# dfm/emcee

Measured on AMD Instinct MI355X. Metric: walker-updates/sec (whole node), 64-dim correlated Gaussian, StretchMove a=2, higher is better.
Workload: dtype f64

## Files before the change

### emcee_amd/csrc/emx.hip

```cpp
#include <hip/hip_runtime.h>

#include <dlfcn.h>

#include <algorithm>
#include <chrono>
#include <cmath>
#include <cstdint>
#include <cstdio>
#include <cstring>
#include <deque>
#include <mutex>
#include <string>
#include <type_traits>
#include <vector>

#include "../../include/emx.h"
#include "emx_internal.hpp"
#include "emx_kernels.hpp"
#include "emx_launch.hpp"
#include "emx_mtdev.hpp"
#include "emx_mtjump.hpp"
#include "emx_mtpipe.hpp"
#include "emx_walkkde.hpp"
#include "emx_rng.hpp"
// ... 287 lines not shown
    } ring[PLAN_RING + MTDEV_SLOTS];
    MtPlanPipeline* pipe = nullptr;
    int64_t pipe_taken = 0;
    int pipe_ring0 = 0;
    int pipe_nsinks = PIPE_SINKS;
    std::deque<int64_t> pipe_uploads;
    bool pipe_defer = false;
    std::vector<std::pair<int64_t, int>> pipe_deferred;
    hipEvent_t pipe_batch_ev[8] = {};
    int pipe_batch_n = 0, pipe_cons_n = 0;
    unsigned long long* pipe_done = nullptr;
    unsigned* pipe_arrived = nullptr;
    hipStream_t up_stream = nullptr;
    int64_t tune_mt_device_finish = 1;
    int64_t tune_persist_exact_mix = 1;
    int64_t pipe_raw_steps = 0;
    int64_t tune_mt_pipeline = -1;
    MtDevProducer* mtdev = nullptr;
    int64_t mtdev_taken = 0;
    int64_t tune_persist_local = 1;
    int64_t tune_persist_exact_max = 32768;
    int64_t tune_persist_exact_regen_max = 131072;
    int64_t tune_persist_exact_steps = 16;
    int64_t tune_fetch_avoid = 1;
    int64_t tune_fetch_blocks = 64;
    bool pipe_fetch_local = false;
    int64_t tune_fetch_delay_us = 0;
    int64_t tune_persist_span = 1;
    int64_t tune_persist_mix = 1;
    int persist_mix_fits = -1;
    int64_t tune_persist_slab = 1;
    int64_t persist_slab_launches = 0;
    int64_t tune_persist_rows_late = 1;
    int64_t tune_persist_stagger = -1;
    int64_t tune_persist_max_halfsteps = PERSIST_MAX_ITERS;
    int64_t tune_mt_device_min_regen = 786432;
    int64_t tune_mt_regen_min = 16384;
    int64_t pipe_regen_steps = 0;
    int64_t tune_persist_odd = 1;
    int64_t tune_persist_slab_skew = 1;
    int64_t tune_persist_slab_local_max = 4096;
    int64_t call_steps = 1;
    int64_t tune_persist_exact = 1;
    int64_t tune_persist_valu = 1;
    int64_t tune_persist_local_max = 8192;
    int64_t tune_slab = 1;
    int64_t tune_slab_skew = 1;
    int64_t tune_mt_device = 1;
    int64_t tune_mt_device_min = 147456;
    int64_t tune_mt_lookahead = 2;
    int64_t tune_mt_tok_wshift = 11, tune_mt_tok_tail = 2048;
    int64_t mtdev_steps_total = 0, mtdev_starts = 0;
    bool mtdev_defer_release = false;
    int64_t mtdev_release_pending = -1;
    MtDevStats mtdev_stats_last;
    int ring_pos = 0;
    struct Prepared {
        int move, S, slot;
        bool lean;
        int gcol;
        uint64_t step;
        NativeArgs nat;
        double cursor_before;
    };
    std::deque<Prepared> prepared;
    int64_t prep_hint = 1;
// ... 1037 lines not shown
        return 0;
    }
    if (!strcmp(key, "persist_slab_skew")) {
        c->tune_persist_slab_skew = v < 0 ? 0 : (v > 4 ? 4 : v);
        return 0;
    }
    if (!strcmp(key, "persist_slab_local_max_walkers")) {
        c->tune_persist_slab_local_max = v;
        return 0;
    }
    if (!strcmp(key, "persist_odd")) {
        c->tune_persist_odd = v ? 1 : 0;
        return 0;
    }
    if (!strcmp(key, "persist_exact_regen_max_walkers")) {
        PIPE_STOP(c);
        c->tune_persist_exact_regen_max = v;
        return 0;
    }
    if (!strcmp(key, "mt_device_min_walkers_regen")) {
        PIPE_STOP(c);
        c->tune_mt_device_min_regen = v;
        return 0;
    }
    if (!strcmp(key, "mt_regen_min_walkers")) {
        PIPE_STOP(c);
        c->tune_mt_regen_min = v < 0 ? 0 : v;
        return 0;
    }
    if (!strcmp(key, "persist_rows_late")) {
        c->tune_persist_rows_late = v < 0 ? 0 : v > 2 ? 2 : v;
        return 0;
    }
    if (!strcmp(key, "persist_stagger")) {
        c->tune_persist_stagger = v < 0 ? -1 : v > 1279 ? 1279 : v;
        return 0;
    }
    if (!strcmp(key, "persist_max_halfsteps")) {
        c->tune_persist_max_halfsteps = v;
        return 0;
    }
    if (!strcmp(key, "persist_slab")) {
        c->tune_persist_slab = (v == 1 || v == 2) ? v : 0;
        return 0;
    }
    if (!strcmp(key, "persist_local")) {
        c->tune_persist_local = v ? 1 : 0;
        return 0;
    }
    if (!strcmp(key, "persist_exact")) {
        PIPE_STOP(c);
        c->tune_persist_exact = v ? 1 : 0;
        return 0;
    }
    if (!strcmp(key, "persist_exact_max_walkers")) {
        PIPE_STOP(c);
        c->tune_persist_exact_max = v;
        return 0;
    }
    if (!strcmp(key, "persist_exact_steps")) {
        c->tune_persist_exact_steps = std::max<int64_t>(1, std::min<int64_t>(v, 16));
        return 0;
    }
    if (!strcmp(key, "fetch_blocks")) {
        c->tune_fetch_blocks = std::max<int64_t>(0, std::min<int64_t>(v, 65536));
        return 0;
// ... 1628 lines not shown
    const int64_t own = N / nsplits;
    if ((own % 16) != 0) return 0;
    const int64_t tiles = own / 16, per_xcd = std::min<int64_t>(32, std::max<int64_t>(1, cu / 8));
    for (int wpb = 1; wpb <= 8; wpb <<= 1)
        if ((tiles % wpb) == 0 && tiles / wpb <= per_xcd) return tiles / wpb >= 2 ? wpb : 0;
    return 0;
}
static bool persist_local_ok(const emx_ctx* c, const emx_move_desc& m) {
    const bool known = ((m.kind == EMX_MOVE_STRETCH || m.kind == EMX_MOVE_DE) && m.nsplits == 2) || (m.kind == EMX_MOVE_SNOOKER && m.nsplits == 4);
    const int64_t lmax = (c->target == EMX_TARGET_DENSE_GAUSS && c->Dp > 64) ? std::min(c->tune_persist_local_max, c->tune_persist_slab_local_max)
                                                                               : c->tune_persist_local_max;
    return c->tune_persist_local != 0 && known && c->N <= lmax &&
           persist_shape_local_of(c->N, m.nsplits, c->num_cu) != 0;
}
static int persist_shape(const emx_ctx* c, int nsplits) { return persist_shape_of(c->N, nsplits, c->num_cu); }
static bool persist_valu_shape(const Shape& sh) {
    return (sh.G == 8 && (sh.CH == 1 || sh.CH == 2 || sh.CH == 4)) || (sh.G == 4 && sh.CH == 1) || (sh.G == 16 && sh.V == 1 && sh.CH == 4);
}
static bool persist_slab_ok(const emx_ctx* c) {
    if (!c->tune_persist_slab || c->target != EMX_TARGET_DENSE_GAUSS || dense_is_wide(c) || c->Dp < 80 || c->Dp > 128) return false;
    if (c->tune_persist_slab != 2 && c->Dp >= 112 && c->N / 2 / 16 >= 8 * (int64_t)c->num_cu && !(c->D & 1)) return false;
    const Shape sh = pick_shape(c->D, c->Dp);
    return (sh.G == 16 && sh.V == 2 && sh.CH == 4) || (c->tune_persist_odd != 0 && sh.G == 32 && sh.V == 1 && sh.CH == 4);
}

static bool persist_grid_fits(const emx_ctx* cc, const emx_move_desc& m, int wpb) {
    emx_ctx* c = const_cast<emx_ctx*>(cc);
    if (m.kind < 0 || m.kind > 3) return false;
    if (c->persist_fits[m.kind] < 0) {
        const int64_t groups = c->N / m.nsplits / 16 / wpb;
        int per_cu = 0;
        const hipError_t e = c->Dp > 64 ? persist_slab_occupancy(c->Dp / 16, m.kind, c->D & 1, 64 * wpb, slab_lds_bytes(c->Dp, wpb), &per_cu)
                             : (c->D & 1) ? persist_dense_odd_occupancy(c->Dp / 16, m.kind, 64 * wpb, dense_lds_bytes(c->Dp, wpb), &per_cu)
                                        : hot_persist_occupancy(c->Dp / 16, m.kind, 64 * wpb, dense_lds_bytes(c->Dp, wpb), &per_cu);
        c->persist_fits[m.kind] = (e != hipSuccess || (int64_t)per_cu * c->num_cu >= groups) ? 1 : 0;
    }
    return c->persist_fits[m.kind] != 0;
}

static bool persist_valu_wide_ok(const emx_ctx* c, const emx_move_desc& m) {
    const bool known = ((m.kind == EMX_MOVE_STRETCH || m.kind == EMX_MOVE_DE) && m.nsplits == 2) || (m.kind == EMX_MOVE_SNOOKER && m.nsplits == 4);
    const bool valu = c->target == EMX_TARGET_ISO_GAUSS || c->target == EMX_TARGET_DIAG_GAUSS || c->target == EMX_TARGET_ROSENBROCK || c->target == EMX_TARGET_BOX;
    const int64_t nmax = (regen_ctx_ok(c) && m.kind == EMX_MOVE_STRETCH) ? std::max(c->tune_persist_exact_max, c->tune_persist_exact_regen_max) : c->tune_persist_exact_max;
    return known && valu && c->rng_mode == EMX_RNG_MT19937 && c->tune_persist_valu != 0 && c->N <= nmax && persist_shape(c, m.nsplits) != 0;
}

static bool persist_move_ok(const emx_ctx* c, const emx_move_desc& m) {
    const bool known = ((m.kind == EMX_MOVE_STRETCH || m.kind == EMX_MOVE_DE) && m.nsplits == 2) || (m.kind == EMX_MOVE_SNOOKER && m.nsplits == 4);
    if (!known) return false;
    if (c->target == EMX_TARGET_DENSE_GAUSS && c->Dp > 64 && (m.kind == EMX_MOVE_SNOOKER || !persist_slab_ok(c))) return false;
    if (c->target == EMX_TARGET_DENSE_GAUSS && c->Dp > 64 && (c->D & 1) && m.kind != EMX_MOVE_STRETCH) return false;
    if (persist_local_ok(c, m)) return true;
    if (c->target != EMX_TARGET_DENSE_GAUSS) return persist_valu_wide_ok(c, m);
    const int wpb = persist_shape(c, m.nsplits);
    return wpb != 0 && persist_grid_fits(c, m, wpb);
}

static bool persist_mix_member(const emx_move_desc& m) {
    return (m.kind == EMX_MOVE_DE && m.nsplits == 2) || (m.kind == EMX_MOVE_SNOOKER && m.nsplits == 4);
}
static bool persist_mix_local(const emx_ctx* c) {
    for (const auto& m : c->moves)
        if (persist_mix_member(m) && !persist_local_ok(c, m)) return false;
    return persist_shape_local_of(c->N, 2, c->num_cu) != 0;
}
static bool persist_mix_ok(const emx_ctx* cc) {
    emx_ctx* c = const_cast<emx_ctx*>(cc);
// ... 321 lines not shown
        if (mtmode && !devp && c->cur.slot >= 0) used_slots.push_back(c->cur.slot);
        rc = emx_step_end(c);
        if (rc) return rc;
        ++steps;
    }
    if (mtmode && !devp) {
        c->pipe_fetch_local = launch_local;
        const int rcf = pipe_fetch_deferred(c);
        if (rcf) return rcf;
    }
    c->pipe_defer = false;
    if (launch_mix) grid = dim3((unsigned)(c->N / 2 / 16 / c->persist_wpb));
    if (launch_local) grid.x *= 8;
    if (grid.x != c->persist_grid) {
        HIPOK(c, hipMemsetAsync(c->persist_bar, 0, PERSIST_BAR_WORDS * sizeof(unsigned), c->stream));
        c->persist_epoch = 0;
        c->persist_lepoch = 0;
        c->persist_hepoch = 0;
        c->persist_grid = grid.x;
    }
    P.niter = n;
    P.bar = c->persist_bar;
    P.started_host = c->persist_started;
    P.ver = c->persist_ver;
    P.epoch0 = c->persist_epoch + (unsigned)c->tune_persist_test_skew;
    P.lepoch0 = c->persist_lepoch;
    P.hepoch0 = c->persist_hepoch + (unsigned)c->tune_persist_test_skew;
    if (launch_local) {
        c->persist_lepoch += (unsigned)(n - 1);
        c->persist_hepoch += 1u;
    }
    P.timeout_ticks = 100000000ull * (unsigned long long)std::max<int64_t>(1, c->tune_persist_timeout_ms) / 1000ull;
    const bool fam_dense64 = c->target == EMX_TARGET_DENSE_GAUSS && c->Dp <= 64;
    P.stagger = c->tune_persist_stagger >= 0 ? (int32_t)c->tune_persist_stagger
                : (launch_local || store || !fam_dense64) ? 0
                : (launch_mix || launch_move == EMX_MOVE_DE) ? 528
                : launch_move == EMX_MOVE_STRETCH ? 516 : 0;
    c->persist_epoch += (unsigned)n;
    P.seq = ++c->persist_seq;
    lg.seq = P.seq;
    lg.steps = steps;
    if (!mtmode || (!devp && lg.pipe_id != nullptr)) c->plog.push_back(lg);
    hipEvent_t e0 = nullptr, e1 = nullptr;
    const bool prof = c->prof_max > 0 && c->prof_n < c->prof_max;
    if (prof) {
        e0 = c->prof[2 * c->prof_n];
        e1 = c->prof[2 * c->prof_n + 1];
    }
    {
        std::lock_guard<std::mutex> lk(g_persist_mu);
        const int dev = c->device;
        if (dev >= 0 && dev < MAX_DEVICES) {
            if (!g_persist_ev[dev]) HIPOK(c, hipEventCreateWithFlags(&g_persist_ev[dev], hipEventDisableTiming));
            if (g_persist_last[dev] && g_persist_last[dev] != c) HIPOK(c, hipStreamWaitEvent(c->stream, g_persist_ev[dev], 0));
        }
        if (prof) HIPOK(c, hipEventRecord(e0, c->stream));
        hipError_t e;
        const bool rows_late = store && (c->tune_persist_rows_late == 2 ||
                                         (c->tune_persist_rows_late == 1 && (launch_local || c->N / 2 / 16 >= 8 * (int64_t)c->num_cu)));
        if (c->target != EMX_TARGET_DENSE_GAUSS) {
            const Shape shv = pick_shape(c->D, c->D);
            e = launch_persist_valu(shv.G, shv.V, shv.CH, launch_move, launch_local ? 1 : 0, grid, block, c->stream, P);
        } else if (launch_mix) {
            e = launch_persist_mix(c->Dp / 16, launch_local ? 1 : 0, grid, block, lds, c->stream, P);
        } else if (c->Dp > 64) {
            P.base.ablate = c->tune_persist_slab_skew ? 256 | (int32_t)((c->tune_persist_slab_skew - 1) << 9) : 0;
            e = launch_persist_slab(c->Dp / 16, launch_move, launch_local ? 1 : 0, c->D & 1, grid, block, lds, c->stream, P);
            c->persist_slab_launches++;
        } else if (c->D & 1) {
            e = launch_persist_dense_odd(c->Dp / 16, launch_move, launch_local ? 1 : 0, grid, block, lds, c->stream, P);
        } else {
            e = launch_hot_persist_dense(c->Dp / 16, launch_move, launch_local ? 1 : 0, rows_late ? 1 : 0, grid, block, lds, c->stream, P);
        }
        if (launch_local) c->persist_local_launches++;
        if (e != hipSuccess) FAIL(c, -2, "persistent half-step launch failed: %s", hipGetErrorString(e));
        if (prof) {
            HIPOK(c, hipEventRecord(e1, c->stream));
            c->prof_n++;
        }
        if (dev >= 0 && dev < MAX_DEVICES) {
            HIPOK(c, hipEventRecord(g_persist_ev[dev], c->stream));
            g_persist_last[dev] = c;
        }
    }
    if (!used_slots.empty()) {
        hipEvent_t& ev = c->pipe_batch_ev[4 + (c->pipe_cons_n & 3)];
        if (!ev) HIPOK(c, hipEventCreateWithFlags(&ev, hipEventDisableTiming));
        c->pipe_cons_n++;
        HIPOK(c, hipEventRecord(ev, c->stream));
        for (int sl : used_slots) {
            c->ring[sl].consumed_ref = ev;
            c->ring[sl].busy = true;
            c->ring[sl].last_seq = P.seq;
        }
    }
    if (mtmode && !devp) pipe_poll(c);
    c->mtdev_defer_release = false;
    if (c->mtdev_release_pending >= 0 && c->mtdev) {
        const int rcr = c->mtdev->release_batch(c->mtdev_release_pending, c->stream);
        c->mtdev_release_pending = -1;
        if (rcr) FAIL(c, rcr, "%s", c->mtdev->error().c_str());
    }
    c->persist_launches++;
    c->persist_halfsteps += n;
    *done = steps;
// ... 1597 lines not shown
```

### emcee_amd/csrc/emx_hot.hip

```cpp
#include "emx_launch.hpp"

namespace emx {

hipError_t launch_hot_stretch_dense64(int lean, dim3 grid, dim3 block, size_t lds, hipStream_t st, const HalfStepArgs& a) {
    if (lean == 2) return launch_one<8, 2, 4, MOVE_STRETCH, 4, 2>(grid, block, lds, st, a);
    if (lean == 3) return launch_one<8, 2, 4, MOVE_STRETCH, 4, 3>(grid, block, lds, st, a);
    if (lean == 4) return launch_one<8, 2, 4, MOVE_STRETCH, 4, 4>(grid, block, lds, st, a);
    return launch_one<8, 2, 4, MOVE_STRETCH, 4, 1>(grid, block, lds, st, a);
}

template <int G, int V, int CH, int DPB, int MOVE, bool LOCAL = false, bool ROWS_LATE = false>
static hipError_t launch_persist(dim3 grid, dim3 block, size_t lds, hipStream_t st, const PersistArgs& P) {
    auto kern = k_persist<G, V, CH, DPB, MOVE, LOCAL, ROWS_LATE>;
    static size_t lds_granted[MAX_DEVICES] = {};
    int dev = 0;
    if (lds > 48 * 1024 && hipGetDevice(&dev) == hipSuccess && dev >= 0 && dev < MAX_DEVICES && lds > lds_granted[dev]) {
        hipError_t e = hipFuncSetAttribute((const void*)kern, hipFuncAttributeMaxDynamicSharedMemorySize, (int)lds);
        if (e != hipSuccess) return e;
        lds_granted[dev] = lds;
    }
    hipLaunchKernelGGL(kern, grid, block, lds, st, P);
    return hipGetLastError();
}

hipError_t launch_hot_persist_dense(int dpb, int move, int local, int rows_late, dim3 grid, dim3 block, size_t lds, hipStream_t st, const PersistArgs& P) {
    if (rows_late && move == MOVE_STRETCH) {
#define EMX_SCASE(b, ch)                                                                                       \
    if (dpb == b)                                                                                              \
        return local ? launch_persist<8, 2, ch, b, MOVE_STRETCH, true, true>(grid, block, lds, st, P)          \
                     : launch_persist<8, 2, ch, b, MOVE_STRETCH, false, true>(grid, block, lds, st, P);
        EMX_SCASE(1, 1) EMX_SCASE(2, 2) EMX_SCASE(3, 4) EMX_SCASE(4, 4)
#undef EMX_SCASE
        return hipErrorInvalidValue;
    }
    if (local) {
#define EMX_LCASE(b, ch)                                                                                           \
    if (dpb == b)                                                                                                  \
        return move == MOVE_DE        ? launch_persist<8, 2, ch, b, MOVE_DE, true>(grid, block, lds, st, P)        \
               : move == MOVE_SNOOKER ? launch_persist<8, 2, ch, b, MOVE_SNOOKER, true>(grid, block, lds, st, P)   \
                                      : launch_persist<8, 2, ch, b, MOVE_STRETCH, true>(grid, block, lds, st, P);
        EMX_LCASE(1, 1) EMX_LCASE(2, 2) EMX_LCASE(3, 4) EMX_LCASE(4, 4)
#undef EMX_LCASE
        return hipErrorInvalidValue;
    }
#define EMX_CASE(b, ch)                                                                                            \
    if (dpb == b)                                                                                                  \
        return move == MOVE_DE        ? launch_persist<8, 2, ch, b, MOVE_DE>(grid, block, lds, st, P)              \
               : move == MOVE_SNOOKER ? launch_persist<8, 2, ch, b, MOVE_SNOOKER>(grid, block, lds, st, P)         \
                                      : launch_persist<8, 2, ch, b, MOVE_STRETCH>(grid, block, lds, st, P);
    EMX_CASE(1, 1) EMX_CASE(2, 2) EMX_CASE(3, 4) EMX_CASE(4, 4)
#undef EMX_CASE
    return hipErrorInvalidValue;
}

template <int G, int V, int CH, int DPB, int MOVE>
static hipError_t persist_occupancy(int threads, size_t lds, int* per_cu) {
    auto kern = k_persist<G, V, CH, DPB, MOVE>;
    if (lds > 48 * 1024) {
        const hipError_t e = hipFuncSetAttribute((const void*)kern, hipFuncAttributeMaxDynamicSharedMemorySize, (int)lds);
        if (e != hipSuccess) return e;
    }
    return hipOccupancyMaxActiveBlocksPerMultiprocessor(per_cu, kern, threads, lds);
}

hipError_t hot_persist_occupancy(int dpb, int move, int threads, size_t lds, int* per_cu) {
#define EMX_CASE(b, ch)                                                                                     \
    if (dpb == b)                                                                                           \
        return move == MOVE_DE        ? persist_occupancy<8, 2, ch, b, MOVE_DE>(threads, lds, per_cu)       \
               : move == MOVE_SNOOKER ? persist_occupancy<8, 2, ch, b, MOVE_SNOOKER>(threads, lds, per_cu)  \
                                      : persist_occupancy<8, 2, ch, b, MOVE_STRETCH>(threads, lds, per_cu);
    EMX_CASE(1, 1) EMX_CASE(2, 2) EMX_CASE(3, 4) EMX_CASE(4, 4)
#undef EMX_CASE
    return hipErrorInvalidValue;
}

hipError_t launch_hot_persist_gauss(int dpb, dim3 grid, dim3 block, size_t lds, hipStream_t st, const PersistGaussArgs& P) {
#define EMX_CASE(b, ch)                                                                                              \
    if (dpb == b) {                                                                                                  \
        auto kern = k_persist_gauss<8, 2, ch, b>;                                                                    \
        static size_t lds_granted[MAX_DEVICES] = {};                                                                 \
        int dev = 0;                                                                                                 \
        if (lds > 48 * 1024 && hipGetDevice(&dev) == hipSuccess && dev >= 0 && dev < MAX_DEVICES && lds > lds_granted[dev]) { \
            hipError_t e = hipFuncSetAttribute((const void*)kern, hipFuncAttributeMaxDynamicSharedMemorySize, (int)lds); \
            if (e != hipSuccess) return e;                                                                           \
            lds_granted[dev] = lds;                                                                                  \
        }                                                                                                            \
        hipLaunchKernelGGL(kern, grid, block, lds, st, P);                                                           \
        return hipGetLastError();                                                                                    \
    }
    EMX_CASE(1, 1) EMX_CASE(2, 2) EMX_CASE(3, 4) EMX_CASE(4, 4)
#undef EMX_CASE
    return hipErrorInvalidValue;
}

}
```

### emcee_amd/csrc/emx_kernels.hpp

```cpp
#pragma once
#include <hip/hip_runtime.h>

#include <cstdint>

#include "emx_planlog.hpp"
#include "emx_rng.hpp"

#ifndef EMX_OPT_RED4
#define EMX_OPT_RED4 1
#endif
#ifndef EMX_OPT_RTILE
#define EMX_OPT_RTILE 1
#endif
#ifndef EMX_LEAN_FOLD_D
#define EMX_LEAN_FOLD_D 0
#endif
#ifndef EMX_LEAN_FOLD_SPW
#define EMX_LEAN_FOLD_SPW 1
#endif
#ifndef EMX_OPT_SKEW
#define EMX_OPT_SKEW 1
#endif
#ifndef EMX_SNOOKER_BUDGET
#define EMX_SNOOKER_BUDGET 48
// ... 989 lines not shown
    const int base = row * D;
    if constexpr (V == 1) {
        typedef unsigned int emx_u2 __attribute__((ext_vector_type(2)));
#pragma unroll
        for (int c = 0; c < CH; ++c) {
            const int d = c * G + gl;
            if (d < D) {
                const emx_u2 w = __builtin_amdgcn_raw_buffer_load_b64(rsrc, (base + d) * 8, 0, CPOL);
                double t;
                __builtin_memcpy(&t, &w, 8);
                r.x[c][0] = t;
            } else {
                r.x[c][0] = 0.0;
            }
        }
        return;
    }
#pragma unroll
    for (int c = 0; c < CH; ++c) {
        const int d = (c * G + gl) * V;
        if (d + 1 < D) {
            const emx_u4 w = __builtin_amdgcn_raw_buffer_load_b128(rsrc, (base + d) * 8, 0, CPOL);
            double2 t;
            __builtin_memcpy(&t, &w, 16);
            r.x[c][0] = t.x;
            r.x[c][1] = t.y;
        } else {
            r.x[c][0] = 0.0;
            r.x[c][1] = 0.0;
        }
    }
}
template <int G, int V, int CH, int CPOL = EMX_CPOL_SC1>
__device__ __forceinline__ void store_row_agent(const Row<G, V, CH>& r, __amdgpu_buffer_rsrc_t rsrc, int row, int D, int gl) {
    static_assert(V == 2 || V == 1, "two coordinates per lane and chunk (even ndim), or one (odd ndim)");
    const int base = row * D;
    if constexpr (V == 1) {
        typedef unsigned int emx_u2 __attribute__((ext_vector_type(2)));
#pragma unroll
        for (int c = 0; c < CH; ++c) {
            const int d = c * G + gl;
            if (d < D) {
                emx_u2 w;
                const double t = r.x[c][0];
                __builtin_memcpy(&w, &t, 8);
                __builtin_amdgcn_raw_buffer_store_b64(w, rsrc, (base + d) * 8, 0, CPOL);
            }
        }
        return;
    }
#pragma unroll
    for (int c = 0; c < CH; ++c) {
        const int d = (c * G + gl) * V;
        if (d + 1 < D) {
            const double2 t = {r.x[c][0], r.x[c][1]};
            emx_u4 w;
            __builtin_memcpy(&w, &t, 16);
            __builtin_amdgcn_raw_buffer_store_b128(w, rsrc, (base + d) * 8, 0, CPOL);
        }
    }
}
template <typename T>
__device__ __forceinline__ void store_agent(T* p, T v) { __hip_atomic_store(p, v, __ATOMIC_RELAXED, __HIP_MEMORY_SCOPE_AGENT); }
__device__ __forceinline__ double load_agent(const double* p) { return __hip_atomic_load(p, __ATOMIC_RELAXED, __HIP_MEMORY_SCOPE_AGENT); }
__device__ __forceinline__ unsigned load_agent(const unsigned* p) { return __hip_atomic_load(p, __ATOMIC_RELAXED, __HIP_MEMORY_SCOPE_AGENT); }
template <bool LOCAL, typename T>
// ... 142 lines not shown
                    }
                } else {
                    o2 = __hip_atomic_fetch_add(gctr, 1u, __ATOMIC_RELAXED, __HIP_MEMORY_SCOPE_AGENT);
                }
                if (open && o2 == k * 8 - 1) {
                    __hip_atomic_store(go + 4, LOCAL ? (xcc & 15u) + 1u : 0u, __ATOMIC_RELAXED, __HIP_MEMORY_SCOPE_AGENT);
                    __hip_atomic_store(go + 3, P.seq, __ATOMIC_RELAXED, __HIP_MEMORY_SCOPE_AGENT);
                    if (P.started_host) __hip_atomic_store(P.started_host, P.seq, __ATOMIC_RELAXED, __HIP_MEMORY_SCOPE_SYSTEM);
                    __hip_atomic_store(go, k, __ATOMIC_RELAXED, __HIP_MEMORY_SCOPE_AGENT);
                }
            }
            const unsigned long long t0 = wall_clock64();
            for (;;) {
                const unsigned long long v = __hip_atomic_load(reinterpret_cast<unsigned long long*>(go), __ATOMIC_RELAXED, __HIP_MEMORY_SCOPE_AGENT);
                if ((v >> 32) != 0ull) {
                    ok = 0;
                    break;
                }
                if ((int)((unsigned)v - k) >= 0) break;
                if (wall_clock64() - t0 > P.timeout_ticks) {
                    raise_status(P.base.status, ST_EXCHANGE_TIMEOUT);
                    __hip_atomic_store(go + 1, 1u, __ATOMIC_RELAXED, __HIP_MEMORY_SCOPE_AGENT);
                    ok = 0;
                    break;
                }
            }
        }
        ok_s = ok;
    }
    __syncthreads();
    return ok_s != 0;
}

template <int G, int V, int CH, int DPB, int MOVE = MOVE_STRETCH, bool LOCAL = false, bool ROWS_LATE = false>
static __global__ __launch_bounds__(512) void k_persist(const PersistArgs P) {
    static_assert(MOVE == MOVE_STRETCH || MOVE == MOVE_DE || MOVE == MOVE_SNOOKER, "the red / blue moves");
    if (LOCAL && (blockIdx.x & 7u) != 0u) return;
    const unsigned bid = LOCAL ? blockIdx.x >> 3 : blockIdx.x, ngroups = LOCAL ? gridDim.x >> 3 : gridDim.x;
    constexpr int CPOL = EMX_CPOL_SC1;
    constexpr int CPOL_ST = LOCAL ? 0 : EMX_CPOL_SC1;
    constexpr bool DE = MOVE == MOVE_DE || MOVE == MOVE_SNOOKER;
    constexpr bool SN = MOVE == MOVE_SNOOKER;
    constexpr bool DEFER = !DE;
    constexpr int WPW = 64 / G;
    constexpr int PPT = 16 / WPW;
    constexpr int PF = PPT;
    static_assert(EMX_OPT_RTILE && EMX_OPT_RED4, "the persistent kernel is the one-tile-per-batch form");
    constexpr int Dp = DPB * 16, KK = Dp / 4, RT = Dp + 2;
    static_assert(G * V * CH >= Dp, "row layout must cover the padded dimension");
    extern __shared__ __attribute__((aligned(16))) double smem[];
    const HalfStepArgs& A = P.base;
    const int lane = threadIdx.x & 63;
    const int wib = threadIdx.x >> 6;
    const int sub = lane / G;
    const int gl = lane % G;
    const int D = A.D;
    double* Sfrag = smem;
    double* muS = smem + dense_img_doubles(Dp);
    double* tile = muS + Dp + (size_t)wib * (16 * RT + 32);
    double* qfS = tile + 16 * RT;
    double* facS = qfS + 16;
    {
        constexpr int IMG2 = (dense_img_doubles(Dp) + Dp) / 2;
        const double2* img = reinterpret_cast<const double2*>(A.tp1);
        double2* dst = reinterpret_cast<double2*>(smem);
        for (int e = threadIdx.x; e < IMG2; e += blockDim.x) dst[e] = img[e];
    }
    Row<G, V, CH> mu;
    load_row<G, V, CH>(mu, A.tp0, D, gl);
// ... 23 lines not shown
    Row<G, V, CH> xi[PF];
    {
        const PersistCols I(P.it[0], (size_t)P.base.N);
        const int pbase = I.pos0 + t0;
#pragma unroll
        for (int k = 0; k < PF; ++k) {
            const int pos = pbase + k * WPW + sub;
            wi[k] = I.order[pos];
            ja[k] = I.p0[pos];
            if constexpr (DE) jb[k] = I.p1[pos];
            if constexpr (SN) jc[k] = I.p2[pos];
            s0v[k] = SN ? 0.0 : I.s0[pos];
            facv[k] = I.fac[pos];
        }
        my_i = I.order[pbase + myrow];
        my_logu = I.logu[pbase + myrow];
#pragma unroll
        for (int k = 0; k < PF; ++k) load_row_agent<G, V, CH, CPOL>(xi[k], Xr, wi[k], D, gl);
        my_lpo = load_agent(A.lp + my_i);
    }
    Row<G, V, CH> crow[DEFER ? PF : 1];
    int cwi[PF], cmy_i = 0;
    double clp = 0.0;
    double *cchain = nullptr, *cchain_lp = nullptr;
#pragma unroll
    for (int k = 0; k < PF; ++k) {
        if (DEFER || k == 0) crow[DEFER ? k : 0] = xi[k];
        cwi[k] = 0;
    }
    for (int n = 0; n < P.niter; ++n) {
        const PersistCols I(P.it[n], (size_t)P.base.N);
        Row<G, V, CH> xa[PF], xb[DE ? PF : 1], xc[SN ? PF : 1];
        persist_stagger_wait(P.stagger, wib);
#pragma unroll
        for (int k = 0; k < PF; ++k) {
            load_row_agent<G, V, CH, CPOL>(xa[k], Xr, ja[k], D, gl);
            if constexpr (DE) load_row_agent<G, V, CH, CPOL>(xb[k], Xr, jb[k], D, gl);
            if constexpr (SN) load_row_agent<G, V, CH, CPOL>(xc[k], Xr, jc[k], D, gl);
        }
        const bool more = n + 1 < P.niter;
        const PersistCols J(P.it[more ? n + 1 : n], (size_t)P.base.N);
        const bool pre = more && J.split != 0;
        const unsigned stamp = P.epoch0 + (unsigned)n + 1u;
        int wi_n[PF], ja_n[PF], jb_n[DE ? PF : 1], jc_n[SN ? PF : 1], my_i_n;
        double s0_n[PF], fac_n[PF], my_logu_n;
        {
            const int pbase = J.pos0 + t0;
#pragma unroll
            for (int k = 0; k < PF; ++k) {
                const int pos = pbase + k * WPW + sub;
                wi_n[k] = J.order[pos];
                ja_n[k] = J.p0[pos];
                if constexpr (DE) jb_n[k] = J.p1[pos];
                if constexpr (SN) jc_n[k] = J.p2[pos];
                s0_n[k] = SN ? 0.0 : J.s0[pos];
                fac_n[k] = J.fac[pos];
            }
            my_i_n = J.order[pbase + myrow];
            my_logu_n = J.logu[pbase + myrow];
        }
        if (prof) { asm volatile("s_waitcnt vmcnt(0)" ::: "memory"); }
        EMX_PSTAMP(0);
        Row<G, V, CH> qk[PF];
#pragma unroll
        for (int k = 0; k < PF; ++k) {
            const int srow = k * WPW + sub;
            double factor = facv[k];
            Row<G, V, CH> q;
            make_proposal<G, V, CH, MOVE>(xi[k], xa[k], xb[DE ? k : 0], xc[SN ? k : 0], s0v[k], A.gammas, D, gl, q, factor, ja[k]);
            bool bl = false;
#pragma unroll
            for (int c = 0; c < CH; ++c)
#pragma unroll
                for (int v = 0; v < V; ++v) bl |= !(fabs(q.x[c][v]) <= 1.79769313486231570815e308);
            const bool badq = group_any<G>(bl, sub);
            if (badq && gl == 0) raise_status(A.status, ST_BAD_COORD);
            const int trow = srow & 15;
#pragma unroll
            for (int c = 0; c < CH; ++c)
#pragma unroll
                for (int v = 0; v < V; ++v) {
                    const int d = (c * G + gl) * V + v;
                    if (d < Dp) tile[trow * RT + d] = !badq ? q.x[c][v] - mu.x[c][v] : 0.0;
                }
            qk[k] = q;
            if (gl == 0) facS[trow] = badq ? -__builtin_inf() : factor;
        }
        if (DEFER && cchain) {
#pragma unroll
            for (int k = 0; k < PF; ++k) store_row_stream<G, V, CH>(crow[k], cchain + (size_t)cwi[k] * D, D, gl);
            if (mine) cchain_lp[cmy_i] = clp;
            cchain = nullptr;
        }
        if (I.chain) {
#pragma unroll
            for (int k = 0; k < PF; ++k) {
                if constexpr (DEFER)
                    crow[k] = xi[k];
                else
                    store_row_stream<G, V, CH>(xi[k], I.chain + (size_t)wi[k] * D, D, gl);
            }
        }
        double my_lpo_n = 0.0;
        if (!ROWS_LATE && more) {
#pragma unroll
            for (int k = 0; k < PF; ++k) load_row_agent<G, V, CH, CPOL>(xi[k], Xr, wi_n[k], D, gl);
            my_lpo_n = load_agent(A.lp + my_i_n);
        }
        EMX_WAVE_SYNC();
        EMX_PSTAMP(1);
        double my_qf;
        {
            const int am = lane & 15, ak = lane >> 4;
            typedef double d4 __attribute__((ext_vector_type(4)));
            double afr[KK];
#pragma unroll
            for (int kk = 0; kk < KK; ++kk) afr[kk] = tile[am * RT + 4 * kk + ak];
            double part[4] = {0.0, 0.0, 0.0, 0.0};
#pragma unroll
            for (int nb = 0; nb < DPB; ++nb) {
                d4 accv = {0.0, 0.0, 0.0, 0.0};
#pragma unroll
                for (int kk = 4 * nb; kk < KK; ++kk)
                    accv = __builtin_amdgcn_mfma_f64_16x16x4f64(afr[kk], Sfrag[(dense_block(DPB, nb, kk >> 2) * 4 + (kk & 3)) * 64 + lane], accv, 0, 0, 0);
#pragma unroll
                for (int r = 0; r < 4; ++r) part[r] = fma(accv[r], accv[r], part[r]);
            }
            my_qf = row16_sum4(part[0], part[1], part[2], part[3], lane);
        }
        if (ROWS_LATE && more) {
            __builtin_amdgcn_sched_barrier(0);
#pragma unroll
            for (int k = 0; k < PF; ++k) load_row_agent<G, V, CH, CPOL>(xi[k], Xr, wi_n[k], D, gl);
            my_lpo_n = load_agent(A.lp + my_i_n);
            __builtin_amdgcn_sched_barrier(0);
        }
        if (prof) { asm volatile("s_nop 0" ::: "memory"); }
        EMX_PSTAMP(2);
        bool acc = false;
        if (mine) {
            const double lpn = -0.5 * my_qf;
            if (lpn != lpn) raise_status(A.status, ST_NAN_LOGP);
            const double lnpdiff = facS[myrow] + lpn - my_lpo;
            acc = lnpdiff > my_logu;
            store_scope<LOCAL>(A.acc + my_i, (uint8_t)(acc ? 1 : 0));
            if (acc) {
                store_scope<LOCAL>(A.lp + my_i, lpn);
                store_scope<LOCAL>(P.ver + my_i, stamp);
            }
            if (I.chain_lp) {
                if constexpr (DEFER)
                    clp = acc ? lpn : my_lpo;
                else
                    I.chain_lp[my_i] = acc ? lpn : my_lpo;
                if (acc) store_scope<LOCAL>(A.acc_count + my_i, load_agent(A.acc_count + my_i) + 1u);
            }
        }
        const unsigned long long am64 = __ballot(acc);
#pragma unroll
        for (int pp = 0; pp < PPT; ++pp) {
            const int row = pp * WPW + sub;
            const bool ac = (am64 >> ((row & 3) * 16 + (row >> 2))) & 1ull;
            if (ac) {
                store_row_agent<G, V, CH, CPOL_ST>(qk[pp], Xr, wi[pp], D, gl);
                if (I.chain) {
                    if constexpr (DEFER)
                        crow[pp] = qk[pp];
                    else
                        store_row_stream<G, V, CH>(qk[pp], I.chain + (size_t)wi[pp] * D, D, gl);
                }
            }
        }
        if (DEFER && I.chain) {
            cchain = I.chain;
            cchain_lp = I.chain_lp;
            cmy_i = my_i;
#pragma unroll
// ... 1421 lines not shown
```

### emcee_amd/csrc/emx_launch.hpp

```cpp
#pragma once
#include <hip/hip_runtime.h>

#include "emx_kernels.hpp"

namespace emx {

constexpr int MAX_DEVICES = 64;

template <int G, int V, int CH, int MOVE, int DPB, int LEAN = 0>
hipError_t launch_one(dim3 grid, dim3 block, size_t lds, hipStream_t st, const HalfStepArgs& a) {
    auto kern = k_halfstep<G, V, CH, MOVE, DPB, LEAN>;
    static size_t lds_granted[MAX_DEVICES] = {};
    int dev = 0;
    if (lds > 48 * 1024 && hipGetDevice(&dev) == hipSuccess && dev >= 0 && dev < MAX_DEVICES && lds > lds_granted[dev]) {
        hipError_t e = hipFuncSetAttribute((const void*)kern, hipFuncAttributeMaxDynamicSharedMemorySize, (int)lds);
        if (e != hipSuccess) return e;
        lds_granted[dev] = lds;
    }
    hipLaunchKernelGGL(kern, grid, block, lds, st, a);
    return hipGetLastError();
}

hipError_t launch_hot_stretch_dense64(int lean, dim3 grid, dim3 block, size_t lds, hipStream_t st, const HalfStepArgs& a);
hipError_t launch_hot_persist_dense(int dpb, int move, int local, int rows_late, dim3 grid, dim3 block, size_t lds, hipStream_t st, const PersistArgs& P);
hipError_t hot_persist_occupancy(int dpb, int move, int threads, size_t lds, int* per_cu);
hipError_t launch_hot_persist_gauss(int dpb, dim3 grid, dim3 block, size_t lds, hipStream_t st, const PersistGaussArgs& P);
hipError_t launch_persist_mix(int dpb, int local, dim3 grid, dim3 block, size_t lds, hipStream_t st, const PersistArgs& P);
hipError_t persist_mix_occupancy(int dpb, int threads, size_t lds, int* per_cu);
hipError_t launch_persist_valu(int G, int V, int CH, int move, int local, dim3 grid, dim3 block, hipStream_t st, const PersistArgs& P);
hipError_t launch_slab_dense(int dpb, int move, dim3 grid, dim3 block, size_t lds, hipStream_t st, const HalfStepArgs& a);
size_t slab_lds_bytes(int Dp, int waves);
hipError_t launch_persist_dense_odd(int dpb, int move, int local, dim3 grid, dim3 block, size_t lds, hipStream_t st, const PersistArgs& P);
hipError_t persist_dense_odd_occupancy(int dpb, int move, int threads, size_t lds, int* per_cu);
hipError_t launch_persist_slab(int dpb, int move, int local, int odd, dim3 grid, dim3 block, size_t lds, hipStream_t st, const PersistArgs& P);
hipError_t persist_slab_occupancy(int dpb, int move, int odd, int threads, size_t lds, int* per_cu);

struct WideLpArgs {
    const double* rows;
    const int32_t* order;
    const double* img;
    double* out;
    uint32_t* status;
    const int32_t* t_hi_dev;
    int32_t D, Dp, pos0, t_lo, t_hi, scatter, check_bad;
    int32_t single_role;
};
struct WideCommitArgs {
    double* X;
    double* lp;
    uint8_t* acc;
    uint32_t* acc_count;
    double* chain;
    double* chain_lp;
    double* sendbuf;
    const double* qout;
    const double* fout;
    const double* newlp;
    const int32_t* order;
// ... 11 lines not shown
```

Measured before the change: 3.368 billion.

## Pipeline per-chunk proposal build with MFMA quadratic-form accumulation in persistent dense stretch kernel

```diff
diff --git a/emcee_amd/csrc/emx.hip b/emcee_amd/csrc/emx.hip
--- a/emcee_amd/csrc/emx.hip
+++ b/emcee_amd/csrc/emx.hip
@@ -343,6 +343,7 @@
     int64_t tune_persist_slab = 1;
     int64_t persist_slab_launches = 0;
     int64_t tune_persist_rows_late = 1;
+    int64_t tune_persist_pipe = -1;
     int64_t tune_persist_stagger = -1;
     int64_t tune_persist_max_halfsteps = PERSIST_MAX_ITERS;
     int64_t tune_mt_device_min_regen = 786432;
@@ -1446,6 +1447,11 @@
         c->tune_persist_rows_late = v < 0 ? 0 : v > 2 ? 2 : v;
         return 0;
     }
+    if (!strcmp(key, "persist_pipe")) {
+        c->tune_persist_pipe = v < 0 ? -1 : v > 1 ? 1 : v;
+        for (auto& f : c->persist_fits) f = -1;
+        return 0;
+    }
     if (!strcmp(key, "persist_stagger")) {
         c->tune_persist_stagger = v < 0 ? -1 : v > 1279 ? 1279 : v;
         return 0;
@@ -3140,7 +3146,7 @@
         int per_cu = 0;
         const hipError_t e = c->Dp > 64 ? persist_slab_occupancy(c->Dp / 16, m.kind, c->D & 1, 64 * wpb, slab_lds_bytes(c->Dp, wpb), &per_cu)
                              : (c->D & 1) ? persist_dense_odd_occupancy(c->Dp / 16, m.kind, 64 * wpb, dense_lds_bytes(c->Dp, wpb), &per_cu)
-                                        : hot_persist_occupancy(c->Dp / 16, m.kind, 64 * wpb, dense_lds_bytes(c->Dp, wpb), &per_cu);
+                                        : hot_persist_occupancy(c->Dp / 16, m.kind, c->tune_persist_pipe != 0, 64 * wpb, dense_lds_bytes(c->Dp, wpb), &per_cu);
         c->persist_fits[m.kind] = (e != hipSuccess || (int64_t)per_cu * c->num_cu >= groups) ? 1 : 0;
     }
     return c->persist_fits[m.kind] != 0;
@@ -3528,6 +3534,11 @@
     }
     P.timeout_ticks = 100000000ull * (unsigned long long)std::max<int64_t>(1, c->tune_persist_timeout_ms) / 1000ull;
     const bool fam_dense64 = c->target == EMX_TARGET_DENSE_GAUSS && c->Dp <= 64;
+    const bool rows_late = store && (c->tune_persist_rows_late == 2 ||
+                                     (c->tune_persist_rows_late == 1 && (launch_local || c->N / 2 / 16 >= 8 * (int64_t)c->num_cu)));
+    const bool pipe_inst = fam_dense64 && !launch_mix && !(c->D & 1) && hot_persist_has_pipe(c->Dp / 16, launch_move, launch_local ? 1 : 0, rows_late ? 1 : 0);
+    const bool pipe = pipe_inst && (c->tune_persist_pipe == 1 ||
+                                    (c->tune_persist_pipe < 0 && !store && c->N / 2 / 16 >= 8 * (int64_t)c->num_cu));
     P.stagger = c->tune_persist_stagger >= 0 ? (int32_t)c->tune_persist_stagger
                 : (launch_local || store || !fam_dense64) ? 0
                 : (launch_mix || launch_move == EMX_MOVE_DE) ? 528
@@ -3552,8 +3563,6 @@
         }
         if (prof) HIPOK(c, hipEventRecord(e0, c->stream));
         hipError_t e;
-        const bool rows_late = store && (c->tune_persist_rows_late == 2 ||
-                                         (c->tune_persist_rows_late == 1 && (launch_local || c->N / 2 / 16 >= 8 * (int64_t)c->num_cu)));
         if (c->target != EMX_TARGET_DENSE_GAUSS) {
             const Shape shv = pick_shape(c->D, c->D);
             e = launch_persist_valu(shv.G, shv.V, shv.CH, launch_move, launch_local ? 1 : 0, grid, block, c->stream, P);
@@ -3566,7 +3575,7 @@
         } else if (c->D & 1) {
             e = launch_persist_dense_odd(c->Dp / 16, launch_move, launch_local ? 1 : 0, grid, block, lds, c->stream, P);
         } else {
-            e = launch_hot_persist_dense(c->Dp / 16, launch_move, launch_local ? 1 : 0, rows_late ? 1 : 0, grid, block, lds, c->stream, P);
+            e = launch_hot_persist_dense(c->Dp / 16, launch_move, launch_local ? 1 : 0, rows_late ? 1 : 0, pipe ? 1 : 0, grid, block, lds, c->stream, P);
         }
         if (launch_local) c->persist_local_launches++;
         if (e != hipSuccess) FAIL(c, -2, "persistent half-step launch failed: %s", hipGetErrorString(e));
diff --git a/emcee_amd/csrc/emx_hot.hip b/emcee_amd/csrc/emx_hot.hip
--- a/emcee_amd/csrc/emx_hot.hip
+++ b/emcee_amd/csrc/emx_hot.hip
@@ -9,9 +9,9 @@
     return launch_one<8, 2, 4, MOVE_STRETCH, 4, 1>(grid, block, lds, st, a);
 }
 
-template <int G, int V, int CH, int DPB, int MOVE, bool LOCAL = false, bool ROWS_LATE = false>
+template <int G, int V, int CH, int DPB, int MOVE, bool LOCAL = false, bool ROWS_LATE = false, bool PIPE = false>
 static hipError_t launch_persist(dim3 grid, dim3 block, size_t lds, hipStream_t st, const PersistArgs& P) {
-    auto kern = k_persist<G, V, CH, DPB, MOVE, LOCAL, ROWS_LATE>;
+    auto kern = k_persist<G, V, CH, DPB, MOVE, LOCAL, ROWS_LATE, PIPE>;
     static size_t lds_granted[MAX_DEVICES] = {};
     int dev = 0;
     if (lds > 48 * 1024 && hipGetDevice(&dev) == hipSuccess && dev >= 0 && dev < MAX_DEVICES && lds > lds_granted[dev]) {
@@ -23,7 +23,13 @@
     return hipGetLastError();
 }
 
-hipError_t launch_hot_persist_dense(int dpb, int move, int local, int rows_late, dim3 grid, dim3 block, size_t lds, hipStream_t st, const PersistArgs& P) {
+bool hot_persist_has_pipe(int dpb, int move, int local, int rows_late) { return dpb == 4 && move == MOVE_STRETCH && !local && !rows_late; }
+
+hipError_t launch_hot_persist_dense(int dpb, int move, int local, int rows_late, int pipe, dim3 grid, dim3 block, size_t lds, hipStream_t st, const PersistArgs& P) {
+    if (pipe) {
+        if (!hot_persist_has_pipe(dpb, move, local, rows_late)) return hipErrorInvalidValue;
+        return launch_persist<8, 2, 4, 4, MOVE_STRETCH, false, false, true>(grid, block, lds, st, P);
+    }
     if (rows_late && move == MOVE_STRETCH) {
 #define EMX_SCASE(b, ch)                                                                                       \
     if (dpb == b)                                                                                              \
@@ -53,9 +59,9 @@
     return hipErrorInvalidValue;
 }
 
-template <int G, int V, int CH, int DPB, int MOVE>
+template <int G, int V, int CH, int DPB, int MOVE, bool PIPE = false>
 static hipError_t persist_occupancy(int threads, size_t lds, int* per_cu) {
-    auto kern = k_persist<G, V, CH, DPB, MOVE>;
+    auto kern = k_persist<G, V, CH, DPB, MOVE, false, false, PIPE>;
     if (lds > 48 * 1024) {
         const hipError_t e = hipFuncSetAttribute((const void*)kern, hipFuncAttributeMaxDynamicSharedMemorySize, (int)lds);
         if (e != hipSuccess) return e;
@@ -63,7 +69,14 @@
     return hipOccupancyMaxActiveBlocksPerMultiprocessor(per_cu, kern, threads, lds);
 }
 
-hipError_t hot_persist_occupancy(int dpb, int move, int threads, size_t lds, int* per_cu) {
+hipError_t hot_persist_occupancy(int dpb, int move, int pipe, int threads, size_t lds, int* per_cu) {
+    if (pipe && hot_persist_has_pipe(dpb, move, 0, 0)) {
+        int a = 0, b = 0;
+        hipError_t e = persist_occupancy<8, 2, 4, 4, MOVE_STRETCH, true>(threads, lds, &a);
+        if (e == hipSuccess) e = persist_occupancy<8, 2, 4, 4, MOVE_STRETCH>(threads, lds, &b);
+        *per_cu = a < b ? a : b;
+        return e;
+    }
 #define EMX_CASE(b, ch)                                                                                     \
     if (dpb == b)                                                                                           \
         return move == MOVE_DE        ? persist_occupancy<8, 2, ch, b, MOVE_DE>(threads, lds, per_cu)       \
diff --git a/emcee_amd/csrc/emx_kernels.hpp b/emcee_amd/csrc/emx_kernels.hpp
--- a/emcee_amd/csrc/emx_kernels.hpp
+++ b/emcee_amd/csrc/emx_kernels.hpp
@@ -1045,6 +1045,21 @@
     }
 }
 template <int G, int V, int CH, int CPOL = EMX_CPOL_SC1>
+__device__ __forceinline__ void load_chunk_agent(Row<G, V, CH>& r, __amdgpu_buffer_rsrc_t rsrc, int row, int D, int gl, int c) {
+    static_assert(V == 2, "two coordinates per lane and chunk");
+    const int d = (c * G + gl) * V;
+    if (d + 1 < D) {
+        const emx_u4 w = __builtin_amdgcn_raw_buffer_load_b128(rsrc, (row * D + d) * 8, 0, CPOL);
+        double2 t;
+        __builtin_memcpy(&t, &w, 16);
+        r.x[c][0] = t.x;
+        r.x[c][1] = t.y;
+    } else {
+        r.x[c][0] = 0.0;
+        r.x[c][1] = 0.0;
+    }
+}
+template <int G, int V, int CH, int CPOL = EMX_CPOL_SC1>
 __device__ __forceinline__ void store_row_agent(const Row<G, V, CH>& r, __amdgpu_buffer_rsrc_t rsrc, int row, int D, int gl) {
     static_assert(V == 2 || V == 1, "two coordinates per lane and chunk (even ndim), or one (odd ndim)");
     const int base = row * D;
@@ -1253,9 +1268,10 @@
     return ok_s != 0;
 }
 
-template <int G, int V, int CH, int DPB, int MOVE = MOVE_STRETCH, bool LOCAL = false, bool ROWS_LATE = false>
+template <int G, int V, int CH, int DPB, int MOVE = MOVE_STRETCH, bool LOCAL = false, bool ROWS_LATE = false, bool PIPE = false>
 static __global__ __launch_bounds__(512) void k_persist(const PersistArgs P) {
     static_assert(MOVE == MOVE_STRETCH || MOVE == MOVE_DE || MOVE == MOVE_SNOOKER, "the red / blue moves");
+    static_assert(!PIPE || (MOVE == MOVE_STRETCH && G == 8 && V == 2 && CH == DPB && !ROWS_LATE), "the chunk-pipelined form: a chunk is a column block");
     if (LOCAL && (blockIdx.x & 7u) != 0u) return;
     const unsigned bid = LOCAL ? blockIdx.x >> 3 : blockIdx.x, ngroups = LOCAL ? gridDim.x >> 3 : gridDim.x;
     constexpr int CPOL = EMX_CPOL_SC1;
@@ -1345,11 +1361,18 @@
         const PersistCols I(P.it[n], (size_t)P.base.N);
         Row<G, V, CH> xa[PF], xb[DE ? PF : 1], xc[SN ? PF : 1];
         persist_stagger_wait(P.stagger, wib);
-#pragma unroll
-        for (int k = 0; k < PF; ++k) {
-            load_row_agent<G, V, CH, CPOL>(xa[k], Xr, ja[k], D, gl);
-            if constexpr (DE) load_row_agent<G, V, CH, CPOL>(xb[k], Xr, jb[k], D, gl);
-            if constexpr (SN) load_row_agent<G, V, CH, CPOL>(xc[k], Xr, jc[k], D, gl);
+        if constexpr (PIPE) {
+#pragma unroll
+            for (int c = 0; c < CH; ++c)
+#pragma unroll
+                for (int k = 0; k < PF; ++k) load_chunk_agent<G, V, CH, CPOL>(xa[k], Xr, ja[k], D, gl, c);
+        } else {
+#pragma unroll
+            for (int k = 0; k < PF; ++k) {
+                load_row_agent<G, V, CH, CPOL>(xa[k], Xr, ja[k], D, gl);
+                if constexpr (DE) load_row_agent<G, V, CH, CPOL>(xb[k], Xr, jb[k], D, gl);
+                if constexpr (SN) load_row_agent<G, V, CH, CPOL>(xc[k], Xr, jc[k], D, gl);
+            }
         }
         const bool more = n + 1 < P.niter;
         const PersistCols J(P.it[more ? n + 1 : n], (size_t)P.base.N);
@@ -1375,29 +1398,80 @@
         if (prof) { asm volatile("s_waitcnt vmcnt(0)" ::: "memory"); }
         EMX_PSTAMP(0);
         Row<G, V, CH> qk[PF];
-#pragma unroll
-        for (int k = 0; k < PF; ++k) {
-            const int srow = k * WPW + sub;
-            double factor = facv[k];
-            Row<G, V, CH> q;
-            make_proposal<G, V, CH, MOVE>(xi[k], xa[k], xb[DE ? k : 0], xc[SN ? k : 0], s0v[k], A.gammas, D, gl, q, factor, ja[k]);
-            bool bl = false;
-#pragma unroll
-            for (int c = 0; c < CH; ++c)
-#pragma unroll
-                for (int v = 0; v < V; ++v) bl |= !(fabs(q.x[c][v]) <= 1.79769313486231570815e308);
-            const bool badq = group_any<G>(bl, sub);
-            if (badq && gl == 0) raise_status(A.status, ST_BAD_COORD);
-            const int trow = srow & 15;
-#pragma unroll
-            for (int c = 0; c < CH; ++c)
-#pragma unroll
-                for (int v = 0; v < V; ++v) {
-                    const int d = (c * G + gl) * V + v;
-                    if (d < Dp) tile[trow * RT + d] = !badq ? q.x[c][v] - mu.x[c][v] : 0.0;
+        typedef double pd4 __attribute__((ext_vector_type(4)));
+        pd4 pacc[DPB];
+        bool mybad = false;
+        auto chunk_mfma = [&](int c) {
+            const int am = lane & 15, ak = lane >> 4;
+            double afr[4];
+#pragma unroll
+            for (int i = 0; i < 4; ++i) afr[i] = tile[am * RT + 4 * (4 * c + i) + ak];
+#pragma unroll
+            for (int i = 0; i < 4; ++i)
+#pragma unroll
+                for (int nb = 0; nb <= c; ++nb)
+                    pacc[nb] = __builtin_amdgcn_mfma_f64_16x16x4f64(afr[i], Sfrag[(dense_block(DPB, nb, c) * 4 + i) * 64 + lane], pacc[nb], 0, 0, 0);
+        };
+        if constexpr (PIPE) {
+            bool bl[PF];
+#pragma unroll
+            for (int k = 0; k < PF; ++k) bl[k] = false;
+#pragma unroll
+            for (int nb = 0; nb < DPB; ++nb) pacc[nb] = pd4{0.0, 0.0, 0.0, 0.0};
+#pragma unroll
+            for (int c = 0; c < CH; ++c) {
+#pragma unroll
+                for (int k = 0; k < PF; ++k) {
+                    const int trow = (k * WPW + sub) & 15;
+#pragma unroll
+                    for (int v = 0; v < V; ++v) {
+                        const double diff = xa[k].x[c][v] - xi[k].x[c][v];
+                        const double prod = diff * s0v[k];
+                        const double qv = xa[k].x[c][v] - prod;
+                        qk[k].x[c][v] = qv;
+                        bl[k] |= !(fabs(qv) <= 1.79769313486231570815e308);
+                        tile[trow * RT + (c * G + gl) * V + v] = qv - mu.x[c][v];
+                    }
                 }
-            qk[k] = q;
-            if (gl == 0) facS[trow] = badq ? -__builtin_inf() : factor;
+                if (c < CH - 1) {
+                    EMX_WAVE_SYNC();
+                    chunk_mfma(c);
+                }
+            }
+#pragma unroll
+            for (int k = 0; k < PF; ++k) {
+                const int trow = (k * WPW + sub) & 15;
+                const unsigned long long bm = __ballot(bl[k]);
+                const bool badq = ((bm >> (sub * G)) & ((1ull << G) - 1ull)) != 0ull;
+                if (badq && gl == 0) raise_status(A.status, ST_BAD_COORD);
+                if (gl == 0) facS[trow] = badq ? -__builtin_inf() : facv[k];
+                if (myrow / WPW == k) mybad = ((bm >> ((myrow % WPW) * G)) & ((1ull << G) - 1ull)) != 0ull;
+            }
+        } else {
+#pragma unroll
+            for (int k = 0; k < PF; ++k) {
+                const int srow = k * WPW + sub;
+                double factor = facv[k];
+                Row<G, V, CH> q;
+                make_proposal<G, V, CH, MOVE>(xi[k], xa[k], xb[DE ? k : 0], xc[SN ? k : 0], s0v[k], A.gammas, D, gl, q, factor, ja[k]);
+                bool bl = false;
+#pragma unroll
+                for (int c = 0; c < CH; ++c)
+#pragma unroll
+                    for (int v = 0; v < V; ++v) bl |= !(fabs(q.x[c][v]) <= 1.79769313486231570815e308);
+                const bool badq = group_any<G>(bl, sub);
+                if (badq && gl == 0) raise_status(A.status, ST_BAD_COORD);
+                const int trow = srow & 15;
+#pragma unroll
+                for (int c = 0; c < CH; ++c)
+#pragma unroll
+                    for (int v = 0; v < V; ++v) {
+                        const int d = (c * G + gl) * V + v;
+                        if (d < Dp) tile[trow * RT + d] = !badq ? q.x[c][v] - mu.x[c][v] : 0.0;
+                    }
+                qk[k] = q;
+                if (gl == 0) facS[trow] = badq ? -__builtin_inf() : factor;
+            }
         }
         if (DEFER && cchain) {
 #pragma unroll
@@ -1420,26 +1494,38 @@
             for (int k = 0; k < PF; ++k) load_row_agent<G, V, CH, CPOL>(xi[k], Xr, wi_n[k], D, gl);
             my_lpo_n = load_agent(A.lp + my_i_n);
         }
-        EMX_WAVE_SYNC();
-        EMX_PSTAMP(1);
         double my_qf;
-        {
-            const int am = lane & 15, ak = lane >> 4;
-            typedef double d4 __attribute__((ext_vector_type(4)));
-            double afr[KK];
-#pragma unroll
-            for (int kk = 0; kk < KK; ++kk) afr[kk] = tile[am * RT + 4 * kk + ak];
+        if constexpr (PIPE) {
+            EMX_WAVE_SYNC();
+            EMX_PSTAMP(1);
+            chunk_mfma(CH - 1);
             double part[4] = {0.0, 0.0, 0.0, 0.0};
 #pragma unroll
-            for (int nb = 0; nb < DPB; ++nb) {
-                d4 accv = {0.0, 0.0, 0.0, 0.0};
-#pragma unroll
-                for (int kk = 4 * nb; kk < KK; ++kk)
-                    accv = __builtin_amdgcn_mfma_f64_16x16x4f64(afr[kk], Sfrag[(dense_block(DPB, nb, kk >> 2) * 4 + (kk & 3)) * 64 + lane], accv, 0, 0, 0);
-#pragma unroll
-                for (int r = 0; r < 4; ++r) part[r] = fma(accv[r], accv[r], part[r]);
-            }
+            for (int nb = 0; nb < DPB; ++nb)
+#pragma unroll
+                for (int r = 0; r < 4; ++r) part[r] = fma(pacc[nb][r], pacc[nb][r], part[r]);
             my_qf = row16_sum4(part[0], part[1], part[2], part[3], lane);
+        } else {
+            EMX_WAVE_SYNC();
+            EMX_PSTAMP(1);
+            {
+                const int am = lane & 15, ak = lane >> 4;
+                typedef double d4 __attribute__((ext_vector_type(4)));
+                double afr[KK];
+#pragma unroll
+                for (int kk = 0; kk < KK; ++kk) afr[kk] = tile[am * RT + 4 * kk + ak];
+                double part[4] = {0.0, 0.0, 0.0, 0.0};
+#pragma unroll
+                for (int nb = 0; nb < DPB; ++nb) {
+                    d4 accv = {0.0, 0.0, 0.0, 0.0};
+#pragma unroll
+                    for (int kk = 4 * nb; kk < KK; ++kk)
+                        accv = __builtin_amdgcn_mfma_f64_16x16x4f64(afr[kk], Sfrag[(dense_block(DPB, nb, kk >> 2) * 4 + (kk & 3)) * 64 + lane], accv, 0, 0, 0);
+#pragma unroll
+                    for (int r = 0; r < 4; ++r) part[r] = fma(accv[r], accv[r], part[r]);
+                }
+                my_qf = row16_sum4(part[0], part[1], part[2], part[3], lane);
+            }
         }
         if (ROWS_LATE && more) {
             __builtin_amdgcn_sched_barrier(0);
@@ -1453,9 +1539,9 @@
         bool acc = false;
         if (mine) {
             const double lpn = -0.5 * my_qf;
-            if (lpn != lpn) raise_status(A.status, ST_NAN_LOGP);
+            if (lpn != lpn && !(PIPE && mybad)) raise_status(A.status, ST_NAN_LOGP);
             const double lnpdiff = facS[myrow] + lpn - my_lpo;
-            acc = lnpdiff > my_logu;
+            acc = lnpdiff > my_logu && !(PIPE && mybad);
             store_scope<LOCAL>(A.acc + my_i, (uint8_t)(acc ? 1 : 0));
             if (acc) {
                 store_scope<LOCAL>(A.lp + my_i, lpn);
diff --git a/emcee_amd/csrc/emx_launch.hpp b/emcee_amd/csrc/emx_launch.hpp
--- a/emcee_amd/csrc/emx_launch.hpp
+++ b/emcee_amd/csrc/emx_launch.hpp
@@ -22,8 +22,9 @@
 }
 
 hipError_t launch_hot_stretch_dense64(int lean, dim3 grid, dim3 block, size_t lds, hipStream_t st, const HalfStepArgs& a);
-hipError_t launch_hot_persist_dense(int dpb, int move, int local, int rows_late, dim3 grid, dim3 block, size_t lds, hipStream_t st, const PersistArgs& P);
-hipError_t hot_persist_occupancy(int dpb, int move, int threads, size_t lds, int* per_cu);
+bool hot_persist_has_pipe(int dpb, int move, int local, int rows_late);
+hipError_t launch_hot_persist_dense(int dpb, int move, int local, int rows_late, int pipe, dim3 grid, dim3 block, size_t lds, hipStream_t st, const PersistArgs& P);
+hipError_t hot_persist_occupancy(int dpb, int move, int pipe, int threads, size_t lds, int* per_cu);
 hipError_t launch_hot_persist_gauss(int dpb, dim3 grid, dim3 block, size_t lds, hipStream_t st, const PersistGaussArgs& P);
 hipError_t launch_persist_mix(int dpb, int local, dim3 grid, dim3 block, size_t lds, hipStream_t st, const PersistArgs& P);
 hipError_t persist_mix_occupancy(int dpb, int threads, size_t lds, int* per_cu);
```

New measurement: 3.244 billion (median of 2 runs). -3.7%, worse.
